# NVlabs/curobo

Hardware: NVIDIA H100
Metric: rollout_cost_grad_evals_per_sec (higher is better)
Workload: dtype f32

## Files before the change

curobo_b200/csrc/cb200_kernels.cu:

```cuda
#include <cuda_runtime.h>
#include <stdio.h>
#include <stdlib.h>
#include <string.h>

#include <algorithm>
#include <cmath>
#include <type_traits>
#include <vector>

#include "../../include/curobo_b200.h"
#include "cb200_blob.h"
#include "cb200_bspline.cuh"
#include "cb200_dynamics.cuh"
#include "cb200_dynamics_tile.cuh"
#include "cb200_launch.h"
#include "cb200_math.cuh"
#include "cb200_mesh.cuh"
#include "cb200_warp.cuh"

using namespace cb200;

namespace {

constexpr int kWarpsPerCta = 8;
constexpr int kMinCtas = 2;

struct FusedArgs {
  cb200_rollout_cfg cfg;
  const float *q, *vel, *acc, *jerk, *dt;
  const unsigned char *blob;
  CuboidSet cuboids;
  VoxelSet voxels;
  const int32_t *env_query_idx;
  const float *goal_position, *goal_quat;
  const int32_t *idxs_goal;
  const float *pose_axes_t, *pose_axes_nt, *pose_tol_t, *pose_tol_nt;
  float *cost, *grad_q, *self_cost, *scene_cost, *pose_cost, *cspace_cost;
  float *grad_vel, *grad_acc, *grad_jerk;
  float *link_pos, *link_quat, *robot_spheres;
  int32_t *pose_goalset_idx;
  int32_t B, H;
  int32_t blob_smem_bytes, eval_floats;
  struct Spline {
    const float *knots, *sp, *sv, *sa, *sj, *gp, *gv, *ga, *gj, *traj_dt;
    const int32_t *start_idx, *goal_idx;
    const uint8_t *implicit;
    float *out_p, *out_v, *out_a, *out_j;
    int32_t n_knots, degree, steps;
  } spl;
  struct Dyn {
    const float *masses_com, *inertias, *gravity;
  } dyn;
  const float *cs_target;
  const int32_t *cs_target_idx;
  const float *cs_target_dofw;
  const float4 *sphere_cfgs;
  int32_t n_sphere_cfgs;
  int32_t *work_counter;
  MeshSet meshes;
  const float *cur_pos, *cur_vel, *cur_dt;
  const int32_t *cur_idx;
};

__device__ __forceinline__ const float4 *row_sphere_cfg(const FusedArgs &a, int b, int S) {
  if (a.sphere_cfgs == nullptr) return nullptr;
  int cfg = a.env_query_idx != nullptr ? __ldg(a.env_query_idx + b) : 0;
  if (cfg < 0 || cfg >= a.n_sphere_cfgs) cfg = 0;
  return a.sphere_cfgs + (size_t)cfg * S;
}

__device__ __forceinline__ void cspace_target_term(const FusedArgs &a, int b, int h, int d, int D, float x, float &cost,
                                                   float &gp) {
  const cb200_rollout_cfg &c = a.cfg;
  if (a.cs_target == nullptr) return;
  float tw = c.cspace_target_weight;
  const float dofw = a.cs_target_dofw != nullptr ? __ldg(a.cs_target_dofw + d) : 1.0f;
  if (c.cspace_type == 2) {
    if (h < a.H - 1) tw *= c.cspace_non_terminal_weight_factor;
// ... 346 lines not shown
  const int env = (a.env_query_idx != nullptr) ? __ldg(a.env_query_idx + b) : 0;
  const float sdt = (SWEEP && cfg.use_speed_metric && (a.dt != nullptr || a.spl.knots != nullptr))
                        ? (a.spl.knots != nullptr ? __ldg(a.spl.traj_dt + __ldg(a.spl.goal_idx)) : __ldg(a.dt))
                        : 0.0f;
  CuboidCull cc{0, 0, false};
  if (has_cuboids<SCENE>(a, do_scene)) {
    if (cuboid_cull_state(a, rv, env, !SWEEP, cc)) {
      cuboid_cull_masks(a, rv, es, cc.ce, cc.ncub, lane, W);
      row_sync<W>();
    }
  }
#pragma unroll 1
  for (int s = lane; s < S; s += W) {
    V3 g = mk3(0, 0, 0);
    float c = 0.0f;
    if (do_scene) {
      if (!SWEEP) {
        c = sphere_discrete_terms<SCENE>(a, rv, es, cc, env, s, g);
      } else {
        const float4 sp = es.sph[s];
        const V3 cen = mk3(sp.x, sp.y, sp.z);
        V3 pv = cen, nx = cen;
        if (prev_sph != nullptr) {
          const float4 t = prev_sph[s];
          pv = mk3(t.x, t.y, t.z);
        }
        if (next_sph != nullptr) {
          const float4 t = next_sph[s];
          nx = mk3(t.x, t.y, t.z);
        }
        c = sphere_scene_swept<SCENE & 3>(cen, sp.w, cfg.scene_activation, cfg.scene_weight, prev_sph != nullptr, pv,
                                          next_sph != nullptr, nx, a.cuboids, a.voxels, env, g);
        if (SCENE & 4) {
          const float4 m = mesh_terms(&a.meshes, cfg.scene_activation, cfg.scene_weight, cen, sp.w, env, true, prev_sph != nullptr,
                                      pv, next_sph != nullptr, nx);
          c += m.w;
          g = g + mk3(m.x, m.y, m.z);
        }
        if (cfg.use_speed_metric && prev_sph != nullptr && next_sph != nullptr) speed_metric(pv, cen, nx, sdt, c, g);
      }
    }
    if (GRAD) {
      es.gsph[s] = make_float4(g.x, g.y, g.z, 0.0f);
      r.nnz += (g.x != 0.0f || g.y != 0.0f || g.z != 0.0f) ? 1 : 0;
    }
    r.scene_c += c;
    if (a.scene_cost) a.scene_cost[(size_t)e * S + s] = c;
  }
  row_sync<W>();
  if (GRAD) r.nnz = (int)row_reduce<W, 0>((unsigned)r.nnz) + 2;
  return r;
}

template <bool SMALL = false, int W = 32, bool GRAD = true>
__device__ __forceinline__ void row_phase_b2(const FusedArgs &a, const RobotView &rv, const EvalSmem &es,
                                             const unsigned char *smem_blob, int lane, int e, const RowB1 &r,
                                             float cs_cost, float pose_c) {
  if (GRAD) {
    if (r.fmax > 0.0f && lane == 0) {
      const float4 pi = es.sph[r.bi], pj = es.sph[r.bj];
      const float w = a.cfg.self_weight;
      float4 gi = es.gsph[r.bi], gj = es.gsph[r.bj];
      const float gx = w * (pj.x - pi.x), gy = w * (pj.y - pi.y), gz = w * (pj.z - pi.z);
      gi.x += gx;
      gi.y += gy;
      gi.z += gz;
      gj.x -= gx;
      gj.y -= gy;
      gj.z -= gz;
      es.gsph[r.bi] = gi;
      es.gsph[r.bj] = gj;
    }
    row_sync<W>();
    float *gq = a.grad_q + (size_t)e * rv.D;
    if (!warp_fk_backward_sparse<SMALL, W>(rv, es, lane, gq, r.nnz)) warp_fk_backward_cold<W>(smem_blob, a.blob, es.cumul, lane, gq);
  }
  const float tot = warp_sum<W>(cs_cost + pose_c + r.scene_c) + r.self_c;
  if (lane == 0) a.cost[e] = tot;
  row_sync<W>();
}

__device__ __forceinline__ int next_warp_unit(int32_t *counter, int u, int stride, bool leader) {
  if (counter == nullptr) return u + stride;
  int nxt = 0;
  if (leader) nxt = stride + atomicAdd(counter, 1);
  return __shfl_sync(kFull, nxt, 0);
}
__device__ __forceinline__ void rearm_ticket_counter(int32_t *counter, int workers) {
  __threadfence();
  if (atomicAdd(counter + 1, 1) == workers - 1) {
    counter[0] = 0;
    counter[1] = 0;
  }
}

template <int SCENE, bool SPLINE, int MINB = kMinCtas, int ROWS = 1>
__global__ void __launch_bounds__(kWarpsPerCta * 32, MINB) rollout_fused_kernel(const __grid_constant__ FusedArgs a) {
  static_assert(ROWS == 1 || (ROWS == 2 && MINB == 3 && !SPLINE), "paired rows: arm build only");
  constexpr int W = 32 / ROWS;
  CB200_EXTERN_SHARED __align__(128) unsigned char smem[];
  __shared__ unsigned long long mbar;
  stage_blob_to_smem(smem, a.blob, (uint32_t)a.blob_smem_bytes, &mbar);
  const int warp = threadIdx.x >> 5, lane = threadIdx.x & (W - 1), nwarps = blockDim.x >> 5;
  const int half = ROWS == 1 ? 0 : (int)(threadIdx.x >> 4) & 1;
  const bool leader = (threadIdx.x & 31) == 0;
  float *base = reinterpret_cast<float *>(smem + a.blob_smem_bytes) + (size_t)(warp * ROWS + half) * a.eval_floats;
  const int N = a.B * a.H;
  const int stride = gridDim.x * nwarps;
  int u = blockIdx.x * nwarps + warp;
  while (u * ROWS < N) {
    const int e = u * ROWS + half;
    if (ROWS == 1 || e < N) {
      int b = e, h = 0;
      if (a.H != 1) {
        b = e / a.H;
        h = e - b * a.H;
      }
      const RobotView rv = make_robot_view(smem, a.blob);
      const EvalSmem es = carve_eval_smem(base, rv.nl, rv.D, rv.S, rv.L, rv.n_cl);
      float cs_cost = 0.0f, pose_c = 0.0f;
      row_phase_a<SPLINE, W>(a, rv, es, lane, e, b, h, cs_cost, pose_c);
      const RowB1 r = row_phase_b1<false, SCENE, MINB != 3, W>(a, rv, es, lane, e, b, nullptr, nullptr);
      row_phase_b2<MINB == 3, W>(a, rv, es, smem, lane, e, r, cs_cost, pose_c);
    }
    u = next_warp_unit(a.work_counter, u, stride, leader);
  }
  if (a.work_counter != nullptr && leader) rearm_ticket_counter(a.work_counter, stride);
}

template <int SCENE, int MINB = kMinCtas, int ROWS = 1>
__global__ void __launch_bounds__(kWarpsPerCta * 32, MINB) rollout_cost_kernel(const __grid_constant__ FusedArgs a) {
  static_assert(ROWS == 1 || (ROWS == 2 && MINB == 3), "paired rows: arm build only");
  constexpr int W = 32 / ROWS;
  CB200_EXTERN_SHARED __align__(128) unsigned char smem[];
  __shared__ unsigned long long mbar;
  stage_blob_to_smem(smem, a.blob, (uint32_t)a.blob_smem_bytes, &mbar);
  const int warp = threadIdx.x >> 5, lane = threadIdx.x & (W - 1), nwarps = blockDim.x >> 5;
  const int half = ROWS == 1 ? 0 : (int)(threadIdx.x >> 4) & 1;
  const bool leader = (threadIdx.x & 31) == 0;
  float *base = reinterpret_cast<float *>(smem + a.blob_smem_bytes) + (size_t)(warp * ROWS + half) * a.eval_floats;
  const int N = a.B * a.H;
  const int stride = gridDim.x * nwarps;
  int u = blockIdx.x * nwarps + warp;
  while (u * ROWS < N) {
    const int e = u * ROWS + half;
    if (ROWS == 1 || e < N) {
      int b = e, h = 0;
      if (a.H != 1) {
        b = e / a.H;
        h = e - b * a.H;
      }
      const RobotView rv = make_robot_view(smem, a.blob);
      const EvalSmem es = carve_cost_smem(base, rv.nl, rv.D, rv.S, rv.n_cl, rv.n_lp == 0);
      float cs_cost = 0.0f, pose_c = 0.0f;
      row_phase_a<false, W, false>(a, rv, es, lane, e, b, h, cs_cost, pose_c);
      const RowB1 r = row_phase_b1<false, SCENE, MINB != 3, W, false>(a, rv, es, lane, e, b, nullptr, nullptr);
      row_phase_b2<MINB == 3, W, false>(a, rv, es, smem, lane, e, r, cs_cost, pose_c);
    }
    u = next_warp_unit(a.work_counter, u, stride, leader);
  }
  if (a.work_counter != nullptr && leader) rearm_ticket_counter(a.work_counter, stride);
}

constexpr int kBigWarps = 16;

template <int SCENE, bool SMALL = false, bool GRAD = true>
__device__ __forceinline__ RowB1 row_phase_b1_list(const FusedArgs &a, const RobotView &rv, const EvalSmem &es, int lane, int e,
                                                   int b, int &n_list, bool &dense) {
  const cb200_rollout_cfg &cfg = a.cfg;
  const int S = rv.S;
  RowB1 r{0.0f, 0.0f, 0.0f, 0, 0, 0};
  n_list = 0;
  dense = false;
  if (cfg.self_weight > 0.0f && rv.P > 0) {
    r.fmax = warp_self_collision_tiles<false, !SMALL>(rv, es, lane, r.bi, r.bj);
    r.self_c = (r.fmax > 0.0f) ? 0.5f * cfg.self_weight * r.fmax : 0.0f;
  }
  if (a.self_cost && lane == 0) a.self_cost[e] = r.self_c;
// ... 1098 lines not shown
    int per_sm = 0;
    if (cudaOccupancyMaxActiveBlocksPerMultiprocessor(&per_sm, k.kernel, nw * 32, need) != cudaSuccess) continue;
    double score = (double)per_sm * nw;
    if (k.horizon > 0) {
      const int tiles = (k.horizon + nw - 1) / nw;
      score *= (double)k.horizon / ((double)tiles * nw + 0.3 * 2.0 * (tiles - 1));
    }
    if (score > best) {
      best = score;
      p = Plan{nw, per_sm, 0, need};
    }
  }
  return p;
}

Plan plan_team(const PlanKey &k, size_t limit, int team) {
  for (int w = kBigWarps; w >= team; w -= team) {
    const size_t need = k.fixed_bytes + (size_t)(w / team) * k.unit_floats * sizeof(float);
    if (need <= limit) return Plan{w, 0, 0, need};
  }
  return Plan{};
}

Plan plan_dyn(const PlanKey &k, size_t limit) {
  Plan p;
  double best = 0.0;
  for (int nw = kWarpsPerCta; nw >= 1; nw >>= 1) {
    for (int R = 32; R >= 8 && R >= nw; R >>= 1) {
      const size_t need = k.fixed_bytes + (size_t)nw * k.unit_floats * sizeof(float) +
                          (size_t)dyn::tile_floats(k.nl, k.dof, R) * sizeof(float);
      if (need > limit) continue;
      int per_sm = 0;
      if (cudaOccupancyMaxActiveBlocksPerMultiprocessor(&per_sm, k.kernel, nw * 32, need) != cudaSuccess || per_sm < 1) continue;
      const int chunks = (k.horizon + R - 1) / R;
      const double score = (double)per_sm * nw * ((double)k.horizon / ((double)chunks * R)) * (0.75 + 0.25 * R / 32.0);
      if (score > best) {
        best = score;
        p = Plan{nw, per_sm, R, need};
      }
    }
  }
  return p;
}

struct PlanEntry {
  PlanKey key;
  Plan plan;
};
constexpr int kPlanSlots = 16;
thread_local PlanEntry g_plans[kPlanSlots];
thread_local int g_plans_used = 0, g_plans_next = 0;

template <typename F>
cudaError_t cached_plan(const PlanKey &k, const DevInfo &d, F make, Plan &out) {
  for (int i = 0; i < g_plans_used; ++i) {
    if (g_plans[i].key == k) {
      out = g_plans[i].plan;
      return cudaSuccess;
    }
  }
  cudaFuncAttributes fa;
  cudaError_t e = cudaFuncGetAttributes(&fa, k.kernel);
  if (e != cudaSuccess) return e;
  const size_t limit = (size_t)d.max_smem - fa.sharedSizeBytes;
  e = cudaFuncSetAttribute(k.kernel, cudaFuncAttributeMaxDynamicSharedMemorySize, (int)limit);
  if (e != cudaSuccess) return e;
  out = make(k, limit);
  g_plans[g_plans_next] = PlanEntry{k, out};
  g_plans_next = (g_plans_next + 1) % kPlanSlots;
  if (g_plans_used < kPlanSlots) ++g_plans_used;
  return cudaSuccess;
}

int env_int(const char *name, int dflt) {
  const char *s = getenv(name);
  return s ? atoi(s) : dflt;
}

inline CuboidSet to_dev(const cb200_cuboid_set *c) {
  CuboidSet o{};
  if (c != nullptr && c->inv_pose != nullptr && c->max_n > 0)
    o = CuboidSet{c->dims, c->inv_pose, c->enable, c->count, c->max_n, c->num_envs};
  return o;
}
inline VoxelSet to_dev(const cb200_voxel_set *v) {
  VoxelSet o{};
  if (v != nullptr && v->inv_pose != nullptr && v->max_n > 0)
    o = VoxelSet{v->params, v->inv_pose, v->enable, v->count, v->features, v->n_voxels_per_layer,
                 v->max_n,  v->num_envs, v->max_dist, v->mip, v->mip_stride};
  return o;
}

__global__ void voxel_mip_kernel(VoxelSet vs, uint16_t *mip, int n_layers) {
  const long long per = vs.mip_stride;
  for (long long t = (long long)blockIdx.x * blockDim.x + threadIdx.x; t < per * n_layers;
       t += (long long)gridDim.x * blockDim.x) {
    const int k = (int)(t / per);
    long long c = t - (long long)k * per;
    const int nx = (int)vs.params[4 * k + 0], ny = (int)vs.params[4 * k + 1], nz = (int)vs.params[4 * k + 2];
    const int mx = (nx + kMipBlock - 1) >> kMipShift, my = (ny + kMipBlock - 1) >> kMipShift, mz = (nz + kMipBlock - 1) >> kMipShift;
    uint16_t outv = 0x7bffu;
    if (c < (long long)mx * my * mz) {
      const int cz = (int)(c % mz), cy = (int)((c / mz) % my), cx = (int)(c / ((long long)mz * my));
      const uint16_t *feat = vs.features + (size_t)k * vs.n_voxels_per_layer;
      float m = 3.0e38f;
      const int B = kMipBlock;
      const int x1 = min(B * cx + B, nx - 1), y1 = min(B * cy + B, ny - 1), z1 = min(B * cz + B, nz - 1);
      for (int x = B * cx; x <= x1; ++x)
        for (int y = B * cy; y <= y1; ++y)
          for (int z = B * cz; z <= z1; ++z) m = fminf(m, load_half(feat + ((size_t)x * ny + y) * nz + z));
      outv = __half_as_ushort(__float2half_rd(m));
    }
    mip[(size_t)k * per + c] = outv;
  }
}

}

static void bounding_ball(const float *link_spheres, const float *padding, int s_begin, int s_end, float *out, int n_cfg = 1,
// ... 522 lines not shown
      int16_t *cll = reinterpret_cast<int16_t *>(o + h.off_cl_link);
      int16_t *cls = reinterpret_cast<int16_t *>(o + h.off_cl_start);
      float *clb = reinterpret_cast<float *>(o + h.off_cl_bound);
      for (int a = 0; a < n_cl; ++a) {
        cll[a] = (int16_t)cl_link[a];
        cls[a] = (int16_t)cl_start[a];
        bounding_ball(link_spheres, sphere_padding, cl_start[a], cl_start[a + 1], clb + 4 * a, n_cfg, S);
        bounding_ball(link_spheres, nullptr, cl_start[a], cl_start[a + 1],
                      reinterpret_cast<float *>(o + h.off_cl_bound_scene) + 4 * a, n_cfg, S);
      }
      cls[n_cl] = (int16_t)S;
      memcpy(o + h.off_lp, lps.data(), lps.size() * 4);
      for (int s0 = 0; s0 < S; ++s0) o[h.off_sph_cl + s0] = (unsigned char)cl_of_sphere[s0];
    }
  }
  return total;
}

}

struct RolloutShape {
  BlobHeader h;
  long long N;
  int H, scene;
  bool mesh, traj, spline, arm_sized;
  bool dynamics, dynamics_ok;
  int grad_floats, cost_floats;
};

enum class Family { Standard, ArmRows, ArmPairs, Big, Team2, Team4, Traj, TrajDyn };
constexpr int kFamilyVariant[] = {CB200_VARIANT_STANDARD, CB200_VARIANT_ARM,   CB200_VARIANT_ARM,  CB200_VARIANT_BIG,
                                  CB200_VARIANT_TEAM2,    CB200_VARIANT_TEAM4, CB200_VARIANT_TRAJ, CB200_VARIANT_TRAJ_DYN};

template <bool MESH, typename K>
static const void *by_scene(int scene, K k) {
  using std::integral_constant;
  if constexpr (MESH) if (scene == 7) return (const void *)k(integral_constant<int, 7>{});
  const void *const builds[4] = {(const void *)k(integral_constant<int, 0>{}), (const void *)k(integral_constant<int, 1>{}),
                                 (const void *)k(integral_constant<int, 2>{}), (const void *)k(integral_constant<int, 3>{})};
  return scene >= 0 && scene < 4 ? builds[scene] : nullptr;
}

static const void *rollout_kernel(Family f, bool grad, const RolloutShape &r) {
  const int s = r.mesh ? 7 : r.scene;
  switch (f) {
    case Family::Standard:
      if (r.spline) return grad ? by_scene<false>(s, [](auto c) { return rollout_fused_kernel<c, true>; }) : nullptr;
      return by_scene<true>(s, [=](auto c) { return grad ? rollout_fused_kernel<c, false> : rollout_cost_kernel<c>; });
    case Family::ArmRows:
      return by_scene<false>(s, [=](auto c) { return grad ? rollout_fused_kernel<c, false, 3> : rollout_cost_kernel<c, 3>; });
    case Family::ArmPairs:
      if (s > 1) return nullptr;
      if (!grad) return (const void *)(s ? rollout_cost_kernel<1, 3, 2> : rollout_cost_kernel<0, 3, 2>);
      return (const void *)(s ? rollout_fused_kernel<1, false, 3, 2> : rollout_fused_kernel<0, false, 3, 2>);
    case Family::Big:
      if (r.arm_sized)
        return by_scene<true>(s, [=](auto c) { return grad ? rollout_fused_big_kernel<c, true> : rollout_cost_big_kernel<c, true>; });
      return by_scene<true>(s, [=](auto c) { return grad ? rollout_fused_big_kernel<c> : rollout_cost_big_kernel<c>; });
    case Family::Team2: return grad ? by_scene<false>(s, [](auto c) { return rollout_fused_team_kernel<c, 2>; }) : nullptr;
    case Family::Team4: return grad ? by_scene<false>(s, [](auto c) { return rollout_fused_team_kernel<c, 4>; }) : nullptr;
    case Family::Traj:
      if (!grad) return nullptr;
      if (r.spline && r.arm_sized) return by_scene<false>(s, [](auto c) { return rollout_traj_kernel<c, true, true>; });
      if (r.spline) return by_scene<false>(s, [](auto c) { return rollout_traj_kernel<c, true>; });
      if (r.arm_sized) return by_scene<true>(s, [](auto c) { return rollout_traj_kernel<c, false, true>; });
      return by_scene<true>(s, [](auto c) { return rollout_traj_kernel<c, false>; });
    case Family::TrajDyn: return grad ? by_scene<false>(s, [](auto c) { return rollout_traj_dyn_kernel<c>; }) : nullptr;
  }
  return nullptr;
}

struct RolloutPlan { Family family; const void *kernel; int row_floats; Plan plan; };

static cudaError_t select_rollout(const RolloutShape &r, bool grad, const DevInfo &d, RolloutPlan &out) {
  const BlobHeader &h = r.h;
  auto plan = [&](Family f, RolloutPlan &p) {
    const bool team = f == Family::Team2 || f == Family::Team4, dyn = f == Family::TrajDyn;
    const int team_size = f == Family::Team4 ? 4 : 2;
    const int big_floats = grad ? big_smem_floats(h.nl, h.D, h.S, h.L, h.n_cl) : r.cost_floats;
    p.family = f;
    p.kernel = rollout_kernel(f, grad, r);
    p.row_floats = team ? (big_floats + team_extra_floats(team_size, h.nl) + 3) & ~3
                        : f == Family::Big ? big_floats : grad ? r.grad_floats : r.cost_floats;
    const size_t halo_bytes = r.traj ? (size_t)2 * h.S * sizeof(float4) : 0;
    const PlanKey key{p.kernel, d.ordinal, (size_t)h.smem_bytes + halo_bytes, (f == Family::ArmPairs ? 2 : 1) * p.row_floats,
                      r.traj ? r.H : 0, dyn ? h.nl : 0, dyn ? h.D : 0};
    return cached_plan(key, d, [=](const PlanKey &k, size_t limit) {
      if (dyn) return plan_dyn(k, limit);
      return team ? plan_team(k, limit, team_size) : plan_warps(k, limit, f == Family::Big ? kBigWarps : kWarpsPerCta);
    }, p.plan);
  };
  const int big_env = env_int("CB200_BIG", -1);
  const long long slots = (long long)d.sm_count * kBigWarps;
  const bool big_fit = !r.traj && !r.spline && h.n_lp > 0 && h.P > 0;
  const bool big_want = big_env >= 0 ? big_env != 0
                                     : ((size_t)r.grad_floats * sizeof(float) > 8192 ||
                                        ((r.scene & 2) != 0 && (!r.arm_sized || r.N * 2 <= slots)));
  if (big_fit && big_want) {
    RolloutPlan big;
    cudaError_t e = plan(Family::Big, big);
    if (e != cudaSuccess) return e;
    if (grad && !r.mesh && h.nl <= 64) {
      const int team_env = env_int("CB200_TEAM", -1);
      const bool small_robot = (size_t)r.grad_floats * sizeof(float) <= 8192;
      const bool smem_limited = big.plan.nw > 0 && big.plan.nw * big.plan.per_sm < kBigWarps;
      int team = 0;
      if (team_env >= 0) team = team_env;
      else if (small_robot) team = (r.N * 2 <= slots) ? 2 : 0;
      else if (r.N * 4 <= slots) team = 4;
      else if (smem_limited || r.N <= 2 * slots) team = 2;
      if (team == 2 || team == 4) {
        e = plan(team == 4 ? Family::Team4 : Family::Team2, out);
        if (e != cudaSuccess || out.plan.nw > 0) return e;
      }
    }
    if (big.plan.nw > 0) {
      out = big;
      return cudaSuccess;
    }
  }
  if (r.dynamics && !r.dynamics_ok) return cudaErrorInvalidValue;
  Family f = r.dynamics ? Family::TrajDyn : r.traj ? Family::Traj : Family::Standard;
  if (!r.traj && !r.spline && !r.mesh && r.arm_sized) {
    const int pairs_env = env_int("CB200_ARM_PAIRS", -1);
    const bool pairs = h.nl <= 16 && (r.scene & 2) == 0 &&
                       (pairs_env >= 0 ? pairs_env != 0 : 2LL * r.N >= 3LL * d.sm_count * 3 * kWarpsPerCta);
    f = pairs ? Family::ArmPairs : Family::ArmRows;
  }
  const cudaError_t e = plan(f, out);
  if (e != cudaSuccess) return e;
  return out.plan.nw > 0 ? cudaSuccess : cudaErrorInvalidConfiguration;
}

static int prepare_rollout(const cb200_rollout_cfg *cfg, const cb200_rollout_io *io, bool grad, cb200_stream_t stream,
                           FusedArgs &a, RolloutShape &r) {
  if (cfg == nullptr || io == nullptr || io->robot_blob == nullptr || io->cost == nullptr || (grad && io->grad_q == nullptr) ||
      io->batch_size < 0 || io->horizon < 1)
    return ret(cudaErrorInvalidValue);
  if (!grad && (io->q == nullptr || io->spline != nullptr || io->dynamics != nullptr || cfg->use_sweep != 0))
    return ret(cudaErrorInvalidValue);
  const cb200_spline_input *sp = io->spline;
  if (sp == nullptr && io->q == nullptr) return ret(cudaErrorInvalidValue);
  int spline_steps = 0;
  if (sp != nullptr) {
    if (sp->knots == nullptr || sp->start_position == nullptr || sp->start_velocity == nullptr ||
        sp->start_acceleration == nullptr || sp->start_jerk == nullptr || sp->start_idx == nullptr ||
        sp->goal_idx == nullptr || sp->traj_dt == nullptr || sp->use_implicit_goal_state == nullptr ||
        sp->goal_position == nullptr || sp->goal_velocity == nullptr || sp->goal_acceleration == nullptr ||
        sp->goal_jerk == nullptr || sp->n_knots < 1 || sp->degree < 3 || sp->degree > 5)
      return ret(cudaErrorInvalidValue);
    spline_steps = (io->horizon - 1) / (sp->n_knots + sp->degree + 1);
    if (sp->grad_knots != nullptr &&
        (io->grad_vel == nullptr || io->grad_acc == nullptr || io->grad_jerk == nullptr || io->horizon - 1 < 5 ||
         spline_steps < 1 || spline_steps > 32))
      return ret(cudaErrorInvalidValue);
  }
  if (io->goal_position != nullptr && (io->goal_quat == nullptr || cfg->num_goalset < 1)) return ret(cudaErrorInvalidValue);
  r.H = io->horizon;
  r.N = (long long)io->batch_size * io->horizon;
  if (r.N == 0) return ret(cudaSuccess);
  if (io->robot_blob_host == nullptr) return ret(cudaErrorInvalidValue);
  memcpy(&r.h, io->robot_blob_host, sizeof(BlobHeader));
  if (r.h.magic != kBlobMagic || r.h.total_bytes != io->robot_blob_bytes) return ret(cudaErrorInvalidValue);
  const BlobHeader &h = r.h;
  a.cfg = *cfg;
  a.q = io->q;
  a.vel = io->vel;
  a.acc = io->acc;
  a.jerk = io->jerk;
  a.dt = io->dt;
  a.blob = static_cast<const unsigned char *>(io->robot_blob);
  a.cuboids = to_dev(io->cuboids);
  a.voxels = to_dev(io->voxels);
  a.env_query_idx = io->env_query_idx;
  a.goal_position = io->goal_position;
  a.goal_quat = io->goal_quat;
  a.idxs_goal = io->idxs_goal;
  a.pose_axes_t = io->pose_axes_terminal;
  a.pose_axes_nt = io->pose_axes_non_terminal;
// ... 140 lines not shown
```

curobo_b200/csrc/cb200_warp.cuh:

```cuda
#pragma once
#include "cb200_blob.h"
#include "cb200_math.cuh"

namespace cb200 {

constexpr unsigned kFull = 0xffffffffu;

struct RobotView {
  int nl, D, S, L, P, n_levels;
  const float *fixed;
  const float *joff;
  const int16_t *link_map;
  const int16_t *joint_map;
  const int8_t *joint_type;
  const int16_t *tool_map;
  const float4 *spheres;
  const int16_t *sph_link;
  const float *padding;
  const int16_t *link_sph_off;
  const int16_t *link_sph_idx;
  const int16_t *level_off;
  const int16_t *level_links;
  const unsigned long long *anc_mask;
  const int16_t *jl_off;
// ... 14 lines not shown
__device__ __forceinline__ RobotView make_robot_view(const unsigned char *smem_blob, const unsigned char *gmem_blob) {
  const BlobHeader *h = reinterpret_cast<const BlobHeader *>(smem_blob);
  RobotView v;
  v.nl = h->nl;
  v.D = h->D;
  v.S = h->S;
  v.L = h->L;
  v.P = h->P;
  v.n_levels = h->n_levels;
  v.fixed = reinterpret_cast<const float *>(smem_blob + h->off_fixed);
  v.joff = reinterpret_cast<const float *>(smem_blob + h->off_joff);
  v.link_map = reinterpret_cast<const int16_t *>(smem_blob + h->off_link_map);
  v.joint_map = reinterpret_cast<const int16_t *>(smem_blob + h->off_joint_map);
  v.joint_type = reinterpret_cast<const int8_t *>(smem_blob + h->off_joint_type);
  v.tool_map = reinterpret_cast<const int16_t *>(smem_blob + h->off_tool_map);
  v.spheres = reinterpret_cast<const float4 *>(smem_blob + h->off_spheres);
  v.sph_link = reinterpret_cast<const int16_t *>(smem_blob + h->off_sph_link);
  v.padding = reinterpret_cast<const float *>(smem_blob + h->off_padding);
  v.link_sph_off = reinterpret_cast<const int16_t *>(smem_blob + h->off_link_sph_off);
  v.link_sph_idx = reinterpret_cast<const int16_t *>(smem_blob + h->off_link_sph_idx);
  v.level_off = reinterpret_cast<const int16_t *>(smem_blob + h->off_level_off);
  v.level_links = reinterpret_cast<const int16_t *>(smem_blob + h->off_level_links);
  v.anc_mask = reinterpret_cast<const unsigned long long *>(smem_blob + h->off_anc_mask);
  v.jl_off = reinterpret_cast<const int16_t *>(smem_blob + h->off_jl_off);
  v.jl_idx = reinterpret_cast<const int16_t *>(smem_blob + h->off_jl_idx);
  v.limits = reinterpret_cast<const float *>(smem_blob + h->off_limits);
  v.pairs = reinterpret_cast<const uint32_t *>(gmem_blob + h->off_pairs);
  v.n_cl = h->n_cl;
  v.n_lp = h->n_lp;
  v.cl_link = reinterpret_cast<const int16_t *>(smem_blob + h->off_cl_link);
  v.cl_start = reinterpret_cast<const int16_t *>(smem_blob + h->off_cl_start);
  v.cl_bound = reinterpret_cast<const float4 *>(smem_blob + h->off_cl_bound);
  v.lp = reinterpret_cast<const uint32_t *>(smem_blob + h->off_lp);
  v.n_fk_steps = h->n_fk_steps;
  v.fk_sched = reinterpret_cast<const uint32_t *>(smem_blob + h->off_fk_sched);
  v.cl_bound_scene = reinterpret_cast<const float4 *>(smem_blob + h->off_cl_bound_scene);
  v.sph_cl = reinterpret_cast<const uint8_t *>(smem_blob + h->off_sph_cl);
  return v;
}

struct EvalSmem {
  float *cumul;
  float4 *sph;
  float4 *gsph;
  float *ft;
  float *contrib;
  float *qv;
  float *gqv;
  float *pose_g;
  float4 *bc;
  uint32_t *cmask;
  float4 *glist;
};
__host__ __device__ inline int eval_smem_floats(int nl, int D, int S, int L, int n_cl) {
  int n = nl * 12 + S * 8 + nl * 8 + n_cl * 4;
  n += nl + D + D + L * 8 + n_cl;
  return (n + 3) & ~3;
}
__device__ __forceinline__ EvalSmem carve_eval_smem(float *base, int nl, int D, int S, int L, int n_cl) {
  EvalSmem e;
  e.cumul = base;
  e.sph = reinterpret_cast<float4 *>(base + nl * 12);
  e.gsph = e.sph + S;
  e.ft = base + nl * 12 + S * 8;
  e.bc = reinterpret_cast<float4 *>(e.ft + nl * 8);
  e.contrib = e.ft + nl * 8 + n_cl * 4;
  e.qv = e.contrib + nl;
  e.gqv = e.qv + D;
  e.pose_g = e.gqv + D;
  e.cmask = reinterpret_cast<uint32_t *>(e.pose_g + L * 8);
  e.glist = nullptr;
  return e;
}

constexpr int kGradListCap = 96;
__host__ __device__ inline int big_smem_floats(int nl, int D, int S, int L, int n_cl) {
  int n = nl * 12 + S * 4 + nl * 8 + n_cl * 4 + kGradListCap * 4;
  n += nl + D + D + L * 8 + n_cl;
  return (n + 3) & ~3;
}
__device__ __forceinline__ EvalSmem carve_big_smem(float *base, int nl, int D, int S, int L, int n_cl) {
  EvalSmem e;
  e.cumul = base;
  e.sph = reinterpret_cast<float4 *>(base + nl * 12);
  e.gsph = nullptr;
  e.ft = base + nl * 12 + S * 4;
  e.bc = reinterpret_cast<float4 *>(e.ft + nl * 8);
  e.glist = e.bc + n_cl;
  e.contrib = reinterpret_cast<float *>(e.glist + kGradListCap);
  e.qv = e.contrib + nl;
  e.gqv = e.qv + D;
  e.pose_g = e.gqv + D;
  e.cmask = reinterpret_cast<uint32_t *>(e.pose_g + L * 8);
  return e;
}

constexpr int kCullScratchFloats = 16;
__host__ __device__ inline int cost_smem_floats(int nl, int D, int S, int n_cl, bool padded_copy) {
  int n = nl * 12 + S * (padded_copy ? 8 : 4) + kCullScratchFloats + n_cl * 4;
  n += D + n_cl;
  return (n + 3) & ~3;
}
__device__ __forceinline__ EvalSmem carve_cost_smem(float *base, int nl, int D, int S, int n_cl, bool padded_copy) {
  EvalSmem e;
  e.cumul = base;
  e.sph = reinterpret_cast<float4 *>(base + nl * 12);
  e.gsph = padded_copy ? e.sph + S : nullptr;
  e.ft = base + nl * 12 + S * (padded_copy ? 8 : 4);
  e.bc = reinterpret_cast<float4 *>(e.ft + kCullScratchFloats);
  e.qv = reinterpret_cast<float *>(e.bc + n_cl);
  e.cmask = reinterpret_cast<uint32_t *>(e.qv + D);
  e.contrib = e.gqv = e.pose_g = nullptr;
  e.glist = nullptr;
  return e;
}

template <int W>
__device__ __forceinline__ unsigned row_mask() {
  static_assert(W == 32 || W == 16, "a row is a warp or a half-warp");
// ... 255 lines not shown
        if (cb) ib[__popc(mb & lt)] = (unsigned char)lane;
        __syncwarp();
        const int na2 = __popc(ma), nb2 = __popc(mb);
        const float inv_nb2 = 1.0f / (float)nb2;
        #pragma unroll 1
        for (int t = lane; t < na2 * nb2; t += 32) {
          const int io = (int)(((float)t + 0.5f) * inv_nb2);
          const int i = sa + ia[io], j = sb + ib[t - io * nb2];
          const float4 x = padded_sphere<PADDED_COPY>(rv, es, i), y = padded_sphere<PADDED_COPY>(rv, es, j);
          const float rs = x.w + y.w;
          const float dx = x.x - y.x, dy = x.y - y.y, dz = x.z - y.z;
          const float f = rs * rs - (dx * dx + dy * dy + dz * dz);
          if (f > 0.0f) {
            const unsigned long long k = ((unsigned long long)__float_as_uint(f) << 32) |
                                         ((unsigned long long)(0xffffu - (unsigned)i) << 16) | (0xffffu - (unsigned)j);
            key = k > key ? k : key;
          }
        }
        __syncwarp();
        continue;
      }
      const float inv_nb = 1.0f / (float)nb;
      #pragma unroll 1
      for (int t = lane; t < na * nb; t += W) {
        const int io = (int)(((float)t + 0.5f) * inv_nb);
        const int i = sa + io, j = sb + (t - io * nb);
        const float4 x = padded_sphere<PADDED_COPY>(rv, es, i), y = padded_sphere<PADDED_COPY>(rv, es, j);
        const float rs = x.w + y.w;
        const float dx = x.x - y.x, dy = x.y - y.y, dz = x.z - y.z;
        const float f = rs * rs - (dx * dx + dy * dy + dz * dz);
        if (f > 0.0f && x.w >= 0.0f && y.w >= 0.0f) {
          const unsigned long long k = ((unsigned long long)__float_as_uint(f) << 32) |
                                       ((unsigned long long)(0xffffu - (unsigned)i) << 16) | (0xffffu - (unsigned)j);
          key = k > key ? k : key;
        }
      }
    }
  }
#pragma unroll
  for (int o = W / 2; o > 0; o >>= 1) {
    const unsigned long long other = row_shfl_xor<W>(key, o);
    key = other > key ? other : key;
  }
  if (key_out != nullptr) *key_out = key;
  bi = bj = 0;
  if (key == 0ull) return 0.0f;
  bi = 0xffff - (int)((key >> 16) & 0xffffu);
  bj = 0xffff - (int)(key & 0xffffu);
  return __uint_as_float((uint32_t)(key >> 32));
}

template <int W = 32>
__device__ __forceinline__ void warp_fk_upsweep(const RobotView &rv, const EvalSmem &es, int lane, float *gq_out);
template <int W = 32>
__device__ __forceinline__ void warp_fk_backward(const RobotView &rv, const EvalSmem &es, int lane, float *gq_out) {
  #pragma unroll 1
  for (int k = lane; k < rv.nl; k += W) {
    const float *Tk = es.cumul + 12 * k;
    const V3 o = mk3(Tk[3], Tk[7], Tk[11]);
    V3 F = mk3(0, 0, 0), T = mk3(0, 0, 0);
    #pragma unroll 1
    for (int i = rv.link_sph_off[k]; i < rv.link_sph_off[k + 1]; ++i) {
      const int s = rv.link_sph_idx[i];
      const float4 g4 = es.gsph[s];
      const V3 g = mk3(g4.x, g4.y, g4.z);
      if (g.x == 0.0f && g.y == 0.0f && g.z == 0.0f) continue;
      const float4 p4 = es.sph[s];
      F = F + g;
      T = T + cross(mk3(p4.x, p4.y, p4.z) - o, g);
    }
    for (int e = 0; e < rv.L; ++e) {
      if (rv.tool_map[e] != k) continue;
      F = F + mk3(es.pose_g[8 * e + 0], es.pose_g[8 * e + 1], es.pose_g[8 * e + 2]);
      T = T + mk3(es.pose_g[8 * e + 4], es.pose_g[8 * e + 5], es.pose_g[8 * e + 6]);
    }
    float *ft = es.ft + 8 * k;
    ft[0] = F.x;
    ft[1] = F.y;
    ft[2] = F.z;
    ft[4] = T.x;
    ft[5] = T.y;
    ft[6] = T.z;
  }
  row_sync<W>();
  warp_fk_upsweep<W>(rv, es, lane, gq_out);
}

template <int W>
__device__ __forceinline__ void warp_fk_upsweep(const RobotView &rv, const EvalSmem &es, int lane, float *gq_out) {
  #pragma unroll 1
  for (int j = lane; j < rv.nl; j += W) {
    const int jt = rv.joint_type[j];
    float res = 0.0f;
    if (jt >= 0) {
      const float *Tj = es.cumul + 12 * j;
      const V3 oj = mk3(Tj[3], Tj[7], Tj[11]);
      V3 F = mk3(0, 0, 0), T = mk3(0, 0, 0);
      #pragma unroll 1
      for (int k = j; k < rv.nl; ++k) {
        if (!((rv.anc_mask[k] >> j) & 1ull)) continue;
        const float *ft = es.ft + 8 * k;
        const V3 Fk = mk3(ft[0], ft[1], ft[2]);
        const float *Tk = es.cumul + 12 * k;
        const V3 ok = mk3(Tk[3], Tk[7], Tk[11]);
        F = F + Fk;
        T = T + mk3(ft[4], ft[5], ft[6]) + cross(ok - oj, Fk);
      }
      const int ax = (jt >= JT_XR) ? jt - JT_XR : jt;
      const V3 a = mk3(Tj[ax], Tj[4 + ax], Tj[8 + ax]);
      res = rv.joff[2 * j] * ((jt >= JT_XR) ? dot(a, T) : dot(a, F));
    }
    es.contrib[j] = res;
  }
  row_sync<W>();
  for (int d = lane; d < rv.D; d += W) {
    float g = es.gqv[d];
    for (int i = rv.jl_off[d]; i < rv.jl_off[d + 1]; ++i) g += es.contrib[rv.jl_idx[i]];
    gq_out[d] = g;
  }
}

template <int W = 32>
static __device__ __noinline__ void warp_fk_backward_cold(const unsigned char *smem_blob, const unsigned char *gmem_blob,
                                                          float *eval_base, int lane, float *gq_out) {
  const RobotView rv = make_robot_view(smem_blob, gmem_blob);
  const EvalSmem es = carve_eval_smem(eval_base, rv.nl, rv.D, rv.S, rv.L, rv.n_cl);
  warp_fk_backward<W>(rv, es, lane, gq_out);
}

template <bool SMALL = false, int W = 32>
__device__ __forceinline__ bool warp_fk_backward_sparse(const RobotView &rv, const EvalSmem &es, int lane, float *gq_out,
                                                        int nnz) {
  static_assert(W == 32 || SMALL, "half-warp rows take the one-link-per-lane form");
  if (nnz > 2 * rv.nl) return false;
  if (SMALL) {
    float sc = 0.0f;
    V3 ax = mk3(0, 0, 0), og = mk3(0, 0, 0);
    int jt = -1;
    if (lane < rv.nl) {
      jt = rv.joint_type[lane];
      if (jt >= 0) {
        const float *Tj = es.cumul + 12 * lane;
        const int a = (jt >= JT_XR) ? jt - JT_XR : jt;
        ax = mk3(Tj[a], Tj[4 + a], Tj[8 + a]);
        og = mk3(Tj[3], Tj[7], Tj[11]);
        sc = rv.joff[2 * lane];
      }
    }
    float acc = 0.0f;
    const int n_entries = rv.S + rv.L;
#pragma unroll 1
    for (int base = 0; base < n_entries; base += W) {
      const int s = base + lane;
      bool nz = false;
      if (s < rv.S) {
        const float4 g = es.gsph[s];
        nz = (g.x != 0.0f) || (g.y != 0.0f) || (g.z != 0.0f);
      } else if (s < n_entries) {
        const float *pg = es.pose_g + 8 * (s - rv.S);
        nz = pg[0] != 0.0f || pg[1] != 0.0f || pg[2] != 0.0f || pg[4] != 0.0f || pg[5] != 0.0f || pg[6] != 0.0f;
      }
      unsigned m = row_ballot<W>(nz);
      while (m) {
        const int ss = base + __ffs(m) - 1;
        m &= m - 1;
        V3 p, g, om = mk3(0, 0, 0);
        int k;
        if (ss < rv.S) {
          const float4 g4 = es.gsph[ss], p4 = es.sph[ss];
          k = rv.sph_link[ss];
          p = mk3(p4.x, p4.y, p4.z);
          g = mk3(g4.x, g4.y, g4.z);
        } else {
          const float *pg = es.pose_g + 8 * (ss - rv.S);
          k = rv.tool_map[ss - rv.S];
          const float *Tk = es.cumul + 12 * k;
          p = mk3(Tk[3], Tk[7], Tk[11]);
          g = mk3(pg[0], pg[1], pg[2]);
          om = mk3(pg[4], pg[5], pg[6]);
// ... 325 lines not shown
```

Measured before the change: 258.9 million.

## Add dedicated half-warp paired-row gradient kernel with aliased smem and higher occupancy

Replaces the templated paired-row path of the fused kernel with a dedicated rollout_pairs_kernel that runs two rows per warp (16 lanes each), launch-bounded for 4 CTAs per SM. The per-row smem layout aliases the force/torque scratch onto the sphere-gradient buffer, shrinking each row's footprint. The kernel also re-derives views in scoped blocks to cut register pressure and requests the max-shared carveout. The pairs heuristic now picks this path for gradient runs once N exceeds the arm slot count. The aliasing requires the wrench computation to finish reading gradients before any stores, which the extra sync enforces; the scheme risks correctness if that ordering breaks.

Result: faster. 273.4 million, median of 6 (+5.6%).

```diff
diff --git a/curobo_b200/csrc/cb200_kernels.cu b/curobo_b200/csrc/cb200_kernels.cu
--- a/curobo_b200/csrc/cb200_kernels.cu
+++ b/curobo_b200/csrc/cb200_kernels.cu
@@ -24,6 +24,7 @@
 
 constexpr int kWarpsPerCta = 8;
 constexpr int kMinCtas = 2;
+constexpr int kPairCtas = 4;
 
 struct FusedArgs {
   cb200_rollout_cfg cfg;
@@ -476,28 +477,37 @@
   return r;
 }
 
+template <int W = 32>
+__device__ __forceinline__ void row_self_grad(const FusedArgs &a, const EvalSmem &es, int lane, const RowB1 &r) {
+  if (r.fmax > 0.0f && lane == 0) {
+    const float4 pi = es.sph[r.bi], pj = es.sph[r.bj];
+    const float w = a.cfg.self_weight;
+    float4 gi = es.gsph[r.bi], gj = es.gsph[r.bj];
+    const float gx = w * (pj.x - pi.x), gy = w * (pj.y - pi.y), gz = w * (pj.z - pi.z);
+    gi.x += gx;
+    gi.y += gy;
+    gi.z += gz;
+    gj.x -= gx;
+    gj.y -= gy;
+    gj.z -= gz;
+    es.gsph[r.bi] = gi;
+    es.gsph[r.bj] = gj;
+  }
+  row_sync<W>();
+}
+template <bool SMALL = false, int W = 32>
+__device__ __forceinline__ void row_jt_backward(const FusedArgs &a, const RobotView &rv, const EvalSmem &es,
+                                                const unsigned char *smem_blob, int lane, int e, int nnz) {
+  float *gq = a.grad_q + (size_t)e * rv.D;
+  if (!warp_fk_backward_sparse<SMALL, W>(rv, es, lane, gq, nnz)) warp_fk_backward_cold<W>(smem_blob, a.blob, es.cumul, lane, gq);
+}
 template <bool SMALL = false, int W = 32, bool GRAD = true>
 __device__ __forceinline__ void row_phase_b2(const FusedArgs &a, const RobotView &rv, const EvalSmem &es,
                                              const unsigned char *smem_blob, int lane, int e, const RowB1 &r,
                                              float cs_cost, float pose_c) {
   if (GRAD) {
-    if (r.fmax > 0.0f && lane == 0) {
-      const float4 pi = es.sph[r.bi], pj = es.sph[r.bj];
-      const float w = a.cfg.self_weight;
-      float4 gi = es.gsph[r.bi], gj = es.gsph[r.bj];
-      const float gx = w * (pj.x - pi.x), gy = w * (pj.y - pi.y), gz = w * (pj.z - pi.z);
-      gi.x += gx;
-      gi.y += gy;
-      gi.z += gz;
-      gj.x -= gx;
-      gj.y -= gy;
-      gj.z -= gz;
-      es.gsph[r.bi] = gi;
-      es.gsph[r.bj] = gj;
-    }
-    row_sync<W>();
-    float *gq = a.grad_q + (size_t)e * rv.D;
-    if (!warp_fk_backward_sparse<SMALL, W>(rv, es, lane, gq, r.nnz)) warp_fk_backward_cold<W>(smem_blob, a.blob, es.cumul, lane, gq);
+    row_self_grad<W>(a, es, lane, r);
+    row_jt_backward<SMALL, W>(a, rv, es, smem_blob, lane, e, r.nnz);
   }
   const float tot = warp_sum<W>(cs_cost + pose_c + r.scene_c) + r.self_c;
   if (lane == 0) a.cost[e] = tot;
@@ -518,36 +528,92 @@
   }
 }
 
-template <int SCENE, bool SPLINE, int MINB = kMinCtas, int ROWS = 1>
+template <int SCENE, bool SPLINE, int MINB = kMinCtas>
 __global__ void __launch_bounds__(kWarpsPerCta * 32, MINB) rollout_fused_kernel(const __grid_constant__ FusedArgs a) {
-  static_assert(ROWS == 1 || (ROWS == 2 && MINB == 3 && !SPLINE), "paired rows: arm build only");
-  constexpr int W = 32 / ROWS;
   CB200_EXTERN_SHARED __align__(128) unsigned char smem[];
   __shared__ unsigned long long mbar;
   stage_blob_to_smem(smem, a.blob, (uint32_t)a.blob_smem_bytes, &mbar);
-  const int warp = threadIdx.x >> 5, lane = threadIdx.x & (W - 1), nwarps = blockDim.x >> 5;
-  const int half = ROWS == 1 ? 0 : (int)(threadIdx.x >> 4) & 1;
-  const bool leader = (threadIdx.x & 31) == 0;
-  float *base = reinterpret_cast<float *>(smem + a.blob_smem_bytes) + (size_t)(warp * ROWS + half) * a.eval_floats;
+  const int warp = threadIdx.x >> 5, lane = threadIdx.x & 31, nwarps = blockDim.x >> 5;
+  const bool leader = lane == 0;
+  float *base = reinterpret_cast<float *>(smem + a.blob_smem_bytes) + (size_t)warp * a.eval_floats;
   const int N = a.B * a.H;
   const int stride = gridDim.x * nwarps;
-  int u = blockIdx.x * nwarps + warp;
-  while (u * ROWS < N) {
-    const int e = u * ROWS + half;
-    if (ROWS == 1 || e < N) {
+  int e = blockIdx.x * nwarps + warp;
+  while (e < N) {
+    int b = e, h = 0;
+    if (a.H != 1) {
+      b = e / a.H;
+      h = e - b * a.H;
+    }
+    const RobotView rv = make_robot_view(smem, a.blob);
+    const EvalSmem es = carve_eval_smem(base, rv.nl, rv.D, rv.S, rv.L, rv.n_cl);
+    float cs_cost = 0.0f, pose_c = 0.0f;
+    row_phase_a<SPLINE>(a, rv, es, lane, e, b, h, cs_cost, pose_c);
+    const RowB1 r = row_phase_b1<false, SCENE, MINB != 3>(a, rv, es, lane, e, b, nullptr, nullptr);
+    row_phase_b2<MINB == 3>(a, rv, es, smem, lane, e, r, cs_cost, pose_c);
+    e = next_warp_unit(a.work_counter, e, stride, leader);
+  }
+  if (a.work_counter != nullptr && leader) rearm_ticket_counter(a.work_counter, stride);
+}
+
+template <int SCENE>
+__global__ void __launch_bounds__(kWarpsPerCta * 32, kPairCtas) rollout_pairs_kernel(const __grid_constant__ FusedArgs a) {
+  constexpr int W = 16;
+  CB200_EXTERN_SHARED __align__(128) unsigned char smem[];
+  __shared__ unsigned long long mbar;
+  stage_blob_to_smem(smem, a.blob, (uint32_t)a.blob_smem_bytes, &mbar);
+  const int lane = threadIdx.x & (W - 1), nwarps = blockDim.x >> 5;
+  const bool leader = (threadIdx.x & 31) == 0;
+  float *base = reinterpret_cast<float *>(smem + a.blob_smem_bytes) + (size_t)(threadIdx.x >> 4) * a.eval_floats;
+  const int N = a.B * a.H;
+  const int stride = gridDim.x * nwarps;
+  auto row_view = [&] { return make_robot_view(smem, a.blob); };
+  auto row_smem = [&](const RobotView &rv) { return carve_half_row_smem(base, rv.nl, rv.D, rv.S, rv.L, rv.n_cl); };
+  int e = 2 * (blockIdx.x * nwarps + (int)(threadIdx.x >> 5)) + (int)((threadIdx.x >> 4) & 1);
+  while ((e & ~1) < N) {
+    if (e < N) {
       int b = e, h = 0;
       if (a.H != 1) {
         b = e / a.H;
         h = e - b * a.H;
       }
-      const RobotView rv = make_robot_view(smem, a.blob);
-      const EvalSmem es = carve_eval_smem(base, rv.nl, rv.D, rv.S, rv.L, rv.n_cl);
-      float cs_cost = 0.0f, pose_c = 0.0f;
-      row_phase_a<SPLINE, W>(a, rv, es, lane, e, b, h, cs_cost, pose_c);
-      const RowB1 r = row_phase_b1<false, SCENE, MINB != 3, W>(a, rv, es, lane, e, b, nullptr, nullptr);
-      row_phase_b2<MINB == 3, W>(a, rv, es, smem, lane, e, r, cs_cost, pose_c);
-    }
-    u = next_warp_unit(a.work_counter, u, stride, leader);
+      {
+        const RobotView rv = row_view();
+        const EvalSmem es = row_smem(rv);
+        for (int d = lane; d < rv.D; d += W) es.qv[d] = __ldg(a.q + (size_t)e * rv.D + d);
+        row_sync<W>();
+        warp_fk<W>(rv, es, lane);
+        warp_spheres<W>(rv, es, lane, a.robot_spheres ? reinterpret_cast<float4 *>(a.robot_spheres) + (size_t)e * rv.S : nullptr,
+                        row_sphere_cfg(a, b, rv.S));
+      }
+      float row_c;
+      {
+        const RobotView rv = row_view();
+        row_c = row_cspace<false, W>(a, rv, row_smem(rv), lane, e, b, h);
+      }
+      {
+        const RobotView rv = row_view();
+        row_c += row_tool_poses<W>(a, rv, row_smem(rv), lane, e, b, h);
+        row_sync<W>();
+      }
+      RowB1 r;
+      {
+        const RobotView rv = row_view();
+        r = row_phase_b1<false, SCENE, false, W>(a, rv, row_smem(rv), lane, e, b, nullptr, nullptr);
+      }
+      const float tot = warp_sum<W>(row_c + r.scene_c) + ((r.fmax > 0.0f) ? 0.5f * a.cfg.self_weight * r.fmax : 0.0f);
+      {
+        const RobotView rv = row_view();
+        row_self_grad<W>(a, row_smem(rv), lane, r);
+      }
+      {
+        const RobotView rv = row_view();
+        row_jt_backward<true, W>(a, rv, row_smem(rv), smem, lane, e, r.nnz);
+      }
+      if (lane == 0) a.cost[e] = tot;
+      row_sync<W>();
+    }
+    e = 2 * next_warp_unit(a.work_counter, e >> 1, stride, leader) + (e & 1);
   }
   if (a.work_counter != nullptr && leader) rearm_ticket_counter(a.work_counter, stride);
 }
@@ -1752,7 +1818,7 @@
 thread_local int g_plans_used = 0, g_plans_next = 0;
 
 template <typename F>
-cudaError_t cached_plan(const PlanKey &k, const DevInfo &d, F make, Plan &out) {
+cudaError_t cached_plan(const PlanKey &k, const DevInfo &d, F make, Plan &out, bool max_shared = false) {
   for (int i = 0; i < g_plans_used; ++i) {
     if (g_plans[i].key == k) {
       out = g_plans[i].plan;
@@ -1765,6 +1831,12 @@
   const size_t limit = (size_t)d.max_smem - fa.sharedSizeBytes;
   e = cudaFuncSetAttribute(k.kernel, cudaFuncAttributeMaxDynamicSharedMemorySize, (int)limit);
   if (e != cudaSuccess) return e;
+#ifndef CB200_SIMT_EMULATION
+  if (max_shared) {
+    e = cudaFuncSetAttribute(k.kernel, cudaFuncAttributePreferredSharedMemoryCarveout, (int)cudaSharedmemCarveoutMaxShared);
+    if (e != cudaSuccess) return e;
+  }
+#endif
   out = make(k, limit);
   g_plans[g_plans_next] = PlanEntry{k, out};
   g_plans_next = (g_plans_next + 1) % kPlanSlots;
@@ -2393,7 +2465,7 @@
     case Family::ArmPairs:
       if (s > 1) return nullptr;
       if (!grad) return (const void *)(s ? rollout_cost_kernel<1, 3, 2> : rollout_cost_kernel<0, 3, 2>);
-      return (const void *)(s ? rollout_fused_kernel<1, false, 3, 2> : rollout_fused_kernel<0, false, 3, 2>);
+      return (const void *)(s ? rollout_pairs_kernel<1> : rollout_pairs_kernel<0>);
     case Family::Big:
       if (r.arm_sized)
         return by_scene<true>(s, [=](auto c) { return grad ? rollout_fused_big_kernel<c, true> : rollout_cost_big_kernel<c, true>; });
@@ -2422,14 +2494,16 @@
     p.family = f;
     p.kernel = rollout_kernel(f, grad, r);
     p.row_floats = team ? (big_floats + team_extra_floats(team_size, h.nl) + 3) & ~3
-                        : f == Family::Big ? big_floats : grad ? r.grad_floats : r.cost_floats;
+                   : f == Family::Big ? big_floats
+                   : !grad ? r.cost_floats
+                   : f == Family::ArmPairs ? eval_smem_floats(h.nl, h.D, h.S, h.L, h.n_cl, true) : r.grad_floats;
     const size_t halo_bytes = r.traj ? (size_t)2 * h.S * sizeof(float4) : 0;
     const PlanKey key{p.kernel, d.ordinal, (size_t)h.smem_bytes + halo_bytes, (f == Family::ArmPairs ? 2 : 1) * p.row_floats,
                       r.traj ? r.H : 0, dyn ? h.nl : 0, dyn ? h.D : 0};
     return cached_plan(key, d, [=](const PlanKey &k, size_t limit) {
       if (dyn) return plan_dyn(k, limit);
       return team ? plan_team(k, limit, team_size) : plan_warps(k, limit, f == Family::Big ? kBigWarps : kWarpsPerCta);
-    }, p.plan);
+    }, p.plan, f == Family::ArmPairs && grad);
   };
   const int big_env = env_int("CB200_BIG", -1);
   const long long slots = (long long)d.sm_count * kBigWarps;
@@ -2464,8 +2538,9 @@
   Family f = r.dynamics ? Family::TrajDyn : r.traj ? Family::Traj : Family::Standard;
   if (!r.traj && !r.spline && !r.mesh && r.arm_sized) {
     const int pairs_env = env_int("CB200_ARM_PAIRS", -1);
+    const long long arm_slots = (long long)d.sm_count * 3 * kWarpsPerCta;
     const bool pairs = h.nl <= 16 && (r.scene & 2) == 0 &&
-                       (pairs_env >= 0 ? pairs_env != 0 : 2LL * r.N >= 3LL * d.sm_count * 3 * kWarpsPerCta);
+                       (pairs_env >= 0 ? pairs_env != 0 : grad ? r.N > arm_slots : 2LL * r.N >= 3LL * arm_slots);
     f = pairs ? Family::ArmPairs : Family::ArmRows;
   }
   const cudaError_t e = plan(f, out);
diff --git a/curobo_b200/csrc/cb200_warp.cuh b/curobo_b200/csrc/cb200_warp.cuh
--- a/curobo_b200/csrc/cb200_warp.cuh
+++ b/curobo_b200/csrc/cb200_warp.cuh
@@ -90,8 +90,8 @@
   uint32_t *cmask;
   float4 *glist;
 };
-__host__ __device__ inline int eval_smem_floats(int nl, int D, int S, int L, int n_cl) {
-  int n = nl * 12 + S * 8 + nl * 8 + n_cl * 4;
+__host__ __device__ inline int eval_smem_floats(int nl, int D, int S, int L, int n_cl, bool half_row = false) {
+  int n = nl * 12 + S * 8 + (half_row ? 0 : nl * 8) + n_cl * 4;
   n += nl + D + D + L * 8 + n_cl;
   return (n + 3) & ~3;
 }
@@ -103,6 +103,21 @@
   e.ft = base + nl * 12 + S * 8;
   e.bc = reinterpret_cast<float4 *>(e.ft + nl * 8);
   e.contrib = e.ft + nl * 8 + n_cl * 4;
+  e.qv = e.contrib + nl;
+  e.gqv = e.qv + D;
+  e.pose_g = e.gqv + D;
+  e.cmask = reinterpret_cast<uint32_t *>(e.pose_g + L * 8);
+  e.glist = nullptr;
+  return e;
+}
+__device__ __forceinline__ EvalSmem carve_half_row_smem(float *base, int nl, int D, int S, int L, int n_cl) {
+  EvalSmem e;
+  e.cumul = base;
+  e.sph = reinterpret_cast<float4 *>(base + nl * 12);
+  e.gsph = e.sph + S;
+  e.ft = reinterpret_cast<float *>(e.gsph);
+  e.bc = reinterpret_cast<float4 *>(base + nl * 12 + S * 8);
+  e.contrib = reinterpret_cast<float *>(e.bc + n_cl);
   e.qv = e.contrib + nl;
   e.gqv = e.qv + D;
   e.pose_g = e.gqv + D;
@@ -464,35 +479,53 @@
 
 template <int W = 32>
 __device__ __forceinline__ void warp_fk_upsweep(const RobotView &rv, const EvalSmem &es, int lane, float *gq_out);
+__device__ __forceinline__ void link_wrench(const RobotView &rv, const EvalSmem &es, int k, V3 &F, V3 &T) {
+  const float *Tk = es.cumul + 12 * k;
+  const V3 o = mk3(Tk[3], Tk[7], Tk[11]);
+  F = mk3(0, 0, 0);
+  T = mk3(0, 0, 0);
+  #pragma unroll 1
+  for (int i = rv.link_sph_off[k]; i < rv.link_sph_off[k + 1]; ++i) {
+    const int s = rv.link_sph_idx[i];
+    const float4 g4 = es.gsph[s];
+    const V3 g = mk3(g4.x, g4.y, g4.z);
+    if (g.x == 0.0f && g.y == 0.0f && g.z == 0.0f) continue;
+    const float4 p4 = es.sph[s];
+    F = F + g;
+    T = T + cross(mk3(p4.x, p4.y, p4.z) - o, g);
+  }
+  for (int e = 0; e < rv.L; ++e) {
+    if (rv.tool_map[e] != k) continue;
+    F = F + mk3(es.pose_g[8 * e + 0], es.pose_g[8 * e + 1], es.pose_g[8 * e + 2]);
+    T = T + mk3(es.pose_g[8 * e + 4], es.pose_g[8 * e + 5], es.pose_g[8 * e + 6]);
+  }
+}
+__device__ __forceinline__ void store_wrench(const EvalSmem &es, int k, V3 F, V3 T) {
+  float *ft = es.ft + 8 * k;
+  ft[0] = F.x;
+  ft[1] = F.y;
+  ft[2] = F.z;
+  ft[4] = T.x;
+  ft[5] = T.y;
+  ft[6] = T.z;
+}
+
 template <int W = 32>
 __device__ __forceinline__ void warp_fk_backward(const RobotView &rv, const EvalSmem &es, int lane, float *gq_out) {
+  if (W == 16) {
+    V3 F, T;
+    if (lane < rv.nl) link_wrench(rv, es, lane, F, T);
+    row_sync<W>();
+    if (lane < rv.nl) store_wrench(es, lane, F, T);
+    row_sync<W>();
+    warp_fk_upsweep<W>(rv, es, lane, gq_out);
+    return;
+  }
   #pragma unroll 1
   for (int k = lane; k < rv.nl; k += W) {
-    const float *Tk = es.cumul + 12 * k;
-    const V3 o = mk3(Tk[3], Tk[7], Tk[11]);
-    V3 F = mk3(0, 0, 0), T = mk3(0, 0, 0);
-    #pragma unroll 1
-    for (int i = rv.link_sph_off[k]; i < rv.link_sph_off[k + 1]; ++i) {
-      const int s = rv.link_sph_idx[i];
-      const float4 g4 = es.gsph[s];
-      const V3 g = mk3(g4.x, g4.y, g4.z);
-      if (g.x == 0.0f && g.y == 0.0f && g.z == 0.0f) continue;
-      const float4 p4 = es.sph[s];
-      F = F + g;
-      T = T + cross(mk3(p4.x, p4.y, p4.z) - o, g);
-    }
-    for (int e = 0; e < rv.L; ++e) {
-      if (rv.tool_map[e] != k) continue;
-      F = F + mk3(es.pose_g[8 * e + 0], es.pose_g[8 * e + 1], es.pose_g[8 * e + 2]);
-      T = T + mk3(es.pose_g[8 * e + 4], es.pose_g[8 * e + 5], es.pose_g[8 * e + 6]);
-    }
-    float *ft = es.ft + 8 * k;
-    ft[0] = F.x;
-    ft[1] = F.y;
-    ft[2] = F.z;
-    ft[4] = T.x;
-    ft[5] = T.y;
-    ft[6] = T.z;
+    V3 F, T;
+    link_wrench(rv, es, k, F, T);
+    store_wrench(es, k, F, T);
   }
   row_sync<W>();
   warp_fk_upsweep<W>(rv, es, lane, gq_out);
@@ -536,7 +569,8 @@
 static __device__ __noinline__ void warp_fk_backward_cold(const unsigned char *smem_blob, const unsigned char *gmem_blob,
                                                           float *eval_base, int lane, float *gq_out) {
   const RobotView rv = make_robot_view(smem_blob, gmem_blob);
-  const EvalSmem es = carve_eval_smem(eval_base, rv.nl, rv.D, rv.S, rv.L, rv.n_cl);
+  const EvalSmem es = W == 16 ? carve_half_row_smem(eval_base, rv.nl, rv.D, rv.S, rv.L, rv.n_cl)
+                               : carve_eval_smem(eval_base, rv.nl, rv.D, rv.S, rv.L, rv.n_cl);
   warp_fk_backward<W>(rv, es, lane, gq_out);
 }
 
```
